# adelacvg/NS2VC

Measured on AMD Instinct MI355X. Metric: denoiser-steps/sec (10s@24kHz Vocos latent, bs32), higher is better.
Workload: dtype fp16; 1 GPU; 10 s utterance (T=938 Vocos frames), batch 32/GPU, prompt Lp=469, 20-step unipc order 2, hipGraph-captured loop, fp16 MFMA operands; timed job = set_condition + 20 steps; global_batch=32, frames=938, prompt_frames=469, solver=unipc, parallelism=dp1

## Files before the change

### include/ns2vc_hip.h

```cpp
#ifndef NS2VC_HIP_H
#define NS2VC_HIP_H

#include <stddef.h>
#include <stdint.h>

#ifdef __cplusplus
extern "C" {
#endif

#define NS2VC_ABI_VERSION 7
#define NS2VC_MAX_LEVELS 8
#define NS2VC_NCOEF 12

typedef struct ns2vc_unet ns2vc_unet;

typedef struct ns2vc_unet_cfg {
  int32_t latent_channels;
  int32_t content_channels;
  int32_t n_levels;
  int32_t block_out_channels[NS2VC_MAX_LEVELS];
  int32_t norm_num_groups;
  int32_t cross_attention_dim;
  int32_t heads;
  int32_t layers_per_block;
// ... 136 lines not shown
int ns2vc_k_xattn_pack(const void* k, int ldk, const void* v, int ldv, int B, int Lk, int hd, void* out, int precision, void* stream);

typedef struct ns2vc_geglu_args {
  const void* yn; int32_t ldy;
  const float* ln_stats; float ln_eps;
  const void* wstream; const float* consts;
  void* out_op; int32_t ldo;
  int32_t M, dim;
  unsigned* ln_health;
} ns2vc_geglu_args;
int ns2vc_pack_geglu(const float* w1_packed_host, const float* bias1_packed_host, int dim, int precision, void** out_stream_dev, float** out_consts_dev);
int ns2vc_k_geglu(const ns2vc_geglu_args* a, int precision, void* stream);
int ns2vc_pack_geglu_host(const float* w1_packed_host, const float* bias1_packed_host, int dim, int precision, uint16_t* stream_out, float* consts_out);

typedef struct ns2vc_rowchain_args {
  const void* a_op; int32_t lda;
  const void* wstream; const float* bias1; const float* consts2;
  const float* res; int32_t ldres;
  float* out1_f32; int32_t ldo1;
  void* out2_op; int32_t ldo2;
  float ln_eps; int32_t M, dim, n2;
  unsigned* ln_health;
  const float* gn_x; int32_t ldx;
  const long long* gn_stats; const float* gn_gamma; const float* gn_beta;
  float gn_eps; int32_t T, G;
  int32_t slices;
} ns2vc_rowchain_args;
int ns2vc_pack_rowchain(const float* w1_host, const float* w2_host, int dim, int n2, int precision, void** out_stream_dev);
int ns2vc_pack_rowchain_sliced(const float* w1_host, const float* w2_host, int dim, int n2, int slices, int precision, void** out_stream_dev);
int ns2vc_k_rowchain(const ns2vc_rowchain_args* a, int precision, void* stream);
int ns2vc_debug_set_geglu_min_rows(int rows);
int ns2vc_debug_set_attn_keys(int keys);
int ns2vc_debug_set_attn_optimistic(int on);
int ns2vc_debug_set_rowchain_tokens(int nt);

int ns2vc_to_operand(const float* host, size_t n, int precision, void** out_dev);
int ns2vc_from_operand(const void* dev, size_t n, int precision, float* host);
int ns2vc_round_to_operand(const float* host_in, size_t n, int precision, float* host_out);
int ns2vc_pack_weight(const float* rows_host, int N, int K, int precision, void** out_dev);
int ns2vc_k_gemm(const ns2vc_gemm_args* a, int precision, void* stream);
int ns2vc_pack_conv3_tiled(const float* rows_host, int N, int ctot, int c2, int precision, void** out_dev);
int ns2vc_weight_rowsum(const float* rows_host, int N, int K, int precision, float** out_dev);
int ns2vc_debug_set_gemm_trace(void* dev_u64_blocks_x8);
int ns2vc_debug_poison(unsigned pattern, int lds_bytes, void* stream);
int ns2vc_debug_placement(void* stream, int n_blocks, int spin, uint32_t* out_host);
int ns2vc_debug_set_gemm_tile(int bm, int bn, int stages);
int ns2vc_k_attention(const ns2vc_attn_args* a, int head_dim, int precision, void* stream);
int ns2vc_k_groupnorm(const float* a0, int lda0, int c0, const float* a1, int lda1, int c1, int B, int T, int G, float eps,
                      const float* gamma, const float* beta, const float* temb, int ldtemb, int temb_off, int silu,
                      void* out_op, void* raw_op, int precision, void* stream);
int ns2vc_k_groupnorm_stats(const float* a0, int lda0, int c0, const long long* stats0, int B, int T, int G, float eps, const float* gamma,
                            const float* beta, const float* temb, int ldtemb, int temb_off, int silu, void* out_op, int precision, void* stream);
int ns2vc_k_groupnorm_stats2(const float* a0, int lda0, int c0, const long long* stats0, const float* a1, int lda1, int c1, const long long* stats1,
                             int B, int T, int G, float eps, const float* gamma, const float* beta, const float* temb, int ldtemb, int temb_off,
                             int silu, void* out_op, void* raw_op, int precision, void* stream);
int ns2vc_k_layernorm_apply(const float* x, int ldx, int M, int C, float eps, void* out_op, int precision, void* stream);
int ns2vc_k_nct_to_btc(const float* src, int C, int T, int B, float* dst, int ldd, int cpad, void* stream);
int ns2vc_k_btc_to_nct(const float* src, int lds, int C, int T, int B, float* dst, void* stream);
int ns2vc_k_noise(const uint64_t* seeds_dev, int B, int C, int T, int ld, int step, const int32_t* lens_dev, float* out, void* stream);
int ns2vc_k_solver_update(const float* coef_dev, const int32_t* step_dev, const float* x0, float* xe, void* xe_op, int precision, float* xbar,
                          float* d1, float* mprev, float* mprev2, size_t n, int ld, void* stream);

#ifdef __cplusplus
}
#endif
#endif
// ... 1 lines not shown
```

### ns2vc_amd/_lib.py

```python
from __future__ import annotations

import ctypes as C
import os
from typing import Optional

_HERE = os.path.dirname(os.path.abspath(__file__))
LIB_PATH = os.path.join(_HERE, "lib", "libns2vc_hip.so")
NCOEF = 12
MAX_LEVELS = 8
PREC_F32, PREC_BF16, PREC_F16 = 0, 1, 2
ABI_VERSION = 7


class Ns2vcError(RuntimeError):
    pass


class UnetCfg(C.Structure):
    _fields_ = [
        ("latent_channels", C.c_int32), ("content_channels", C.c_int32), ("n_levels", C.c_int32),
        ("block_out_channels", C.c_int32 * MAX_LEVELS), ("norm_num_groups", C.c_int32),
        ("cross_attention_dim", C.c_int32), ("heads", C.c_int32), ("layers_per_block", C.c_int32),
        ("pool_heads", C.c_int32),
    ]
# ... 136 lines not shown
    "ns2vc_dev_sync": (_I, []),
    "ns2vc_stream_create": (_I, [_PP]),
    "ns2vc_stream_create_cu_mask": (_I, [_PP, C.POINTER(C.c_uint32), _I]),
    "ns2vc_stream_destroy": (_I, [_P]),
    "ns2vc_stream_sync": (_I, [_P]),
    "ns2vc_event_create": (_I, [_PP]),
    "ns2vc_event_destroy": (_I, [_P]),
    "ns2vc_event_record": (_I, [_P, _P]),
    "ns2vc_event_elapsed_ms": (_I, [_P, _P, C.POINTER(C.c_float)]),
    "ns2vc_pack_weight": (_I, [_P, _I, _I, _I, _PP]),
    "ns2vc_k_gemm": (_I, [C.POINTER(GemmArgs), _I, _P]),
    "ns2vc_pack_conv3_tiled": (_I, [_P, _I, _I, _I, _I, _PP]),
    "ns2vc_weight_rowsum": (_I, [_P, _I, _I, _I, _PP]),
    "ns2vc_debug_set_gemm_trace": (_I, [_P]),
    "ns2vc_debug_set_gemm_tile": (_I, [_I, _I, _I]),
    "ns2vc_debug_placement": (_I, [_P, _I, _I, C.POINTER(C.c_uint32)]),
    "ns2vc_debug_poison": (_I, [C.c_uint, _I, _P]),
    "ns2vc_k_attention": (_I, [C.POINTER(AttnArgs), _I, _I, _P]),
    "ns2vc_pack_ffn": (_I, [_P, _P, _I, _I, _PP]),
    "ns2vc_pack_ffn_pre": (_I, [_P, _P, _P, _I, _I, _PP]),
    "ns2vc_xattn_pack_bytes": (C.c_size_t, [_I, _I, _I]),
    "ns2vc_k_xattn_pack": (_I, [_P, _I, _P, _I, _I, _I, _I, _P, _I, _P]),
    "ns2vc_k_ffn": (_I, [C.POINTER(FfnArgs), _I, _P]),
    "ns2vc_pack_geglu": (_I, [_P, _P, _I, _I, _PP, _PP]),
    "ns2vc_k_geglu": (_I, [C.POINTER(GegluArgs), _I, _P]),
    "ns2vc_pack_geglu_host": (_I, [_P, _P, _I, _I, _P, _P]),
    "ns2vc_debug_set_geglu_min_rows": (_I, [_I]),
    "ns2vc_pack_rowchain": (_I, [_P, _P, _I, _I, _I, _PP]),
    "ns2vc_pack_rowchain_sliced": (_I, [_P, _P, _I, _I, _I, _I, _PP]),
    "ns2vc_k_rowchain": (_I, [C.POINTER(RowchainArgs), _I, _P]),
    "ns2vc_debug_set_rowchain_tokens": (_I, [_I]),
    "ns2vc_debug_set_attn_keys": (_I, [_I]),
    "ns2vc_debug_set_attn_optimistic": (_I, [_I]),
    "ns2vc_k_groupnorm_stats": (_I, [_P, _I, _I, _P, _I, _I, _I, C.c_float, _P, _P, _P, _I, _I, _I, _P, _I, _P]),
    "ns2vc_k_groupnorm_stats2": (_I, [_P, _I, _I, _P, _P, _I, _I, _P, _I, _I, _I, C.c_float, _P, _P, _P, _I, _I, _I, _P, _P, _I, _P]),
    "ns2vc_k_groupnorm": (_I, [_P, _I, _I, _P, _I, _I, _I, _I, _I, C.c_float, _P, _P, _P, _I, _I, _I, _P, _P, _I, _P]),
    "ns2vc_k_layernorm_apply": (_I, [_P, _I, _I, _I, C.c_float, _P, _I, _P]),
    "ns2vc_to_operand": (_I, [_P, C.c_size_t, _I, _PP]),
    "ns2vc_from_operand": (_I, [_P, C.c_size_t, _I, _P]),
    "ns2vc_round_to_operand": (_I, [_P, C.c_size_t, _I, _P]),
    "ns2vc_k_nct_to_btc": (_I, [_P, _I, _I, _I, _P, _I, _I, _P]),
    "ns2vc_k_btc_to_nct": (_I, [_P, _I, _I, _I, _I, _P, _P]),
    "ns2vc_k_noise": (_I, [_P, _I, _I, _I, _I, _I, _P, _P, _P]),
    "ns2vc_k_solver_update": (_I, [_P, _P, _P, _P, _P, _I, _P, _P, _P, _P, C.c_size_t, _I, _P]),
}

_lib: Optional[C.CDLL] = None


def load(path: Optional[str] = None) -> C.CDLL:
    global _lib
    if _lib is not None and path is None:
        return _lib
    p = path or os.environ.get("NS2VC_LIB") or LIB_PATH
    if not os.path.exists(p):
        raise Ns2vcError(f"{p} not found: the HIP engine is not built. Run __graft_entry__.build() "
                         f"(or `make -C ns2vc_amd/csrc`). There is no CPU fallback.")
    try:
        import torch
    except Exception:
        pass
    lib = C.CDLL(p)
    for name, (res, args) in PROTOTYPES.items():
        fn = getattr(lib, name)
        fn.restype = res
        fn.argtypes = args
# ... 12 lines not shown
```

### ns2vc_amd/csrc/attn.hip

```cpp
#include "common.h"
#include "mma.h"
#include <cstdlib>

namespace ns2vc {

template <typename T> struct AMma;
template <> struct AMma<float> {
  static constexpr int SZ = 4;
  __device__ static __forceinline__ void mma(f32x16_t& acc, const u32x4_t& a, const u32x4_t& b) {
    acc = __builtin_amdgcn_mfma_f32_32x32x2f32(__uint_as_float(a.x), __uint_as_float(b.x), acc, 0, 0, 0);
    acc = __builtin_amdgcn_mfma_f32_32x32x2f32(__uint_as_float(a.y), __uint_as_float(b.y), acc, 0, 0, 0);
    acc = __builtin_amdgcn_mfma_f32_32x32x2f32(__uint_as_float(a.z), __uint_as_float(b.z), acc, 0, 0, 0);
    acc = __builtin_amdgcn_mfma_f32_32x32x2f32(__uint_as_float(a.w), __uint_as_float(b.w), acc, 0, 0, 0);
  }
  __device__ static __forceinline__ f32x16_t mma0(const u32x4_t& a, const u32x4_t& b) {
    f32x16_t acc = __builtin_amdgcn_mfma_f32_32x32x2f32(__uint_as_float(a.x), __uint_as_float(b.x), f32x16_t{0.f, 0.f, 0.f, 0.f, 0.f, 0.f, 0.f, 0.f, 0.f, 0.f, 0.f, 0.f, 0.f, 0.f, 0.f, 0.f}, 0, 0, 0);
    acc = __builtin_amdgcn_mfma_f32_32x32x2f32(__uint_as_float(a.y), __uint_as_float(b.y), acc, 0, 0, 0);
    acc = __builtin_amdgcn_mfma_f32_32x32x2f32(__uint_as_float(a.z), __uint_as_float(b.z), acc, 0, 0, 0);
    acc = __builtin_amdgcn_mfma_f32_32x32x2f32(__uint_as_float(a.w), __uint_as_float(b.w), acc, 0, 0, 0);
    return acc;
  }
  __device__ static __forceinline__ int vpos(int key) { return key; }
};
template <typename TM> struct AMma16 {
  static constexpr int SZ = 2;
  __device__ static __forceinline__ void mma(f32x16_t& acc, const u32x4_t& a, const u32x4_t& b) { MmaT<TM>::mma(acc, a, b); }
  __device__ static __forceinline__ f32x16_t mma0(const u32x4_t& a, const u32x4_t& b) {
    f32x16_t acc = {0.f, 0.f, 0.f, 0.f, 0.f, 0.f, 0.f, 0.f, 0.f, 0.f, 0.f, 0.f, 0.f, 0.f, 0.f, 0.f};
    MmaT<TM>::mma(acc, a, b);
    return acc;
  }
  __device__ static __forceinline__ int vpos(int key) { return (key & ~12) | ((key & 4) << 1) | ((key & 8) >> 1); }
};
template <> struct AMma<bf16_t> : AMma16<bf16_t> {};
template <> struct AMma<f16_t> : AMma16<f16_t> {};

template <typename TM> __device__ __forceinline__ void vt_scatter(char* vp, int rowb, const u32x4_t& v);
template <> __device__ __forceinline__ void vt_scatter<float>(char* vp, int rowb, const u32x4_t& v) {
  *reinterpret_cast<uint32_t*>(vp) = v.x;
  *reinterpret_cast<uint32_t*>(vp + rowb) = v.y;
  *reinterpret_cast<uint32_t*>(vp + 2 * rowb) = v.z;
  *reinterpret_cast<uint32_t*>(vp + 3 * rowb) = v.w;
}
__device__ __forceinline__ void vt_scatter16(char* vp, int rowb, const u32x4_t& v) {
  *reinterpret_cast<uint16_t*>(vp) = (uint16_t)v.x;
  *reinterpret_cast<uint16_t*>(vp + rowb) = (uint16_t)(v.x >> 16);
  *reinterpret_cast<uint16_t*>(vp + 2 * rowb) = (uint16_t)v.y;
  *reinterpret_cast<uint16_t*>(vp + 3 * rowb) = (uint16_t)(v.y >> 16);
  *reinterpret_cast<uint16_t*>(vp + 4 * rowb) = (uint16_t)v.z;
  *reinterpret_cast<uint16_t*>(vp + 5 * rowb) = (uint16_t)(v.z >> 16);
  *reinterpret_cast<uint16_t*>(vp + 6 * rowb) = (uint16_t)v.w;
  *reinterpret_cast<uint16_t*>(vp + 7 * rowb) = (uint16_t)(v.w >> 16);
}
template <> __device__ __forceinline__ void vt_scatter<bf16_t>(char* vp, int rowb, const u32x4_t& v) { vt_scatter16(vp, rowb, v); }
template <> __device__ __forceinline__ void vt_scatter<f16_t>(char* vp, int rowb, const u32x4_t& v) { vt_scatter16(vp, rowb, v); }

__device__ __forceinline__ float half_max(float v) {
  const auto r = __builtin_amdgcn_permlane32_swap(__float_as_uint(v), __float_as_uint(v), false, false);
  return fmaxf(__uint_as_float(r[0]), __uint_as_float(r[1]));
}
__device__ __forceinline__ float half_sum(float v) {
  const auto r = __builtin_amdgcn_permlane32_swap(__float_as_uint(v), __float_as_uint(v), false, false);
  return __uint_as_float(r[0]) + __uint_as_float(r[1]);
}

template <typename TM> __device__ __forceinline__ float round_op(float x);
template <> __device__ __forceinline__ float round_op<float>(float x) { return x; }
template <> __device__ __forceinline__ float round_op<bf16_t>(float x) { return __uint_as_float(pack_bf16x2(0.f, x) & 0xffff0000u); }
template <> __device__ __forceinline__ float round_op<f16_t>(float x) { return f16_lo(pack_f16x2(x, 0.f)); }
template <typename TM> __device__ __forceinline__ u32x4_t aux_chunk(float e0, float e1);
template <> __device__ __forceinline__ u32x4_t aux_chunk<float>(float e0, float e1) { return u32x4_t{__float_as_uint(e0), __float_as_uint(e1), 0u, 0u}; }
template <> __device__ __forceinline__ u32x4_t aux_chunk<bf16_t>(float e0, float e1) { return u32x4_t{pack_bf16x2(e0, e1), 0u, 0u, 0u}; }
template <> __device__ __forceinline__ u32x4_t aux_chunk<f16_t>(float e0, float e1) { return u32x4_t{pack_f16x2(e0, e1), 0u, 0u, 0u}; }
template <typename TM> __device__ __forceinline__ TM op_from_float(float x);
template <> __device__ __forceinline__ float op_from_float<float>(float x) { return x; }
template <> __device__ __forceinline__ bf16_t op_from_float<bf16_t>(float x) { bf16_t r; r.v = (uint16_t)pack_bf16x2(x, 0.f); return r; }
template <> __device__ __forceinline__ f16_t op_from_float<f16_t>(float x) { f16_t r; r.v = (uint16_t)pack_f16x2(x, 0.f); return r; }

__device__ __forceinline__ uint32_t pack_fp8x4(float a, float b, float c, float d) {
  int v = __builtin_amdgcn_cvt_pk_fp8_f32(a, b, 0, false);
  v = __builtin_amdgcn_cvt_pk_fp8_f32(c, d, v, true);
  return (uint32_t)v;
}
typedef int i32x8_t __attribute__((ext_vector_type(8)));
#ifndef NS2VC_ATTN_OPT
#define NS2VC_ATTN_OPT 1
#endif
template <bool B> struct OptTag { static constexpr bool value = B; };
__device__ int g_attn_exact_only = 0;
__device__ __forceinline__ int vpos8(int key) { return ((key & 4) << 3) | ((key & 32) >> 1) | ((key & 24) >> 1) | (key & 3); }
template <typename TM, int HD, int KEYS, bool P8>
__global__ __launch_bounds__(256) void attn_kernel(const AttnArgs a) {
  op_mode_init<TM>();
  static_assert(!P8 || (sizeof(TM) == 2 && KEYS == 64), "the fp8 PV path: 16-bit operand types, one 64-key tile per f8f6f4 MFMA");
  constexpr int NSUB = KEYS / 32;
  constexpr int SZ = AMma<TM>::SZ;
  constexpr int EPC = 16 / SZ;
  constexpr int NS = HD * SZ / 32;
  constexpr int KROWB = HD * SZ + 48;
  constexpr int VSZ = P8 ? 1 : SZ;
  constexpr int VROWB = KEYS * VSZ + 16;
  constexpr int HDX = (HD + 1 + 31) / 32 * 32;
  constexpr int DT = HDX / 32;
  constexpr int NSL = SZ;
  constexpr int KBYTES = KEYS * KROWB, VBYTES = HDX * VROWB;
  constexpr int STAGE = KBYTES + VBYTES;
  constexpr int PPR = HD * SZ / 16;
  constexpr int NPIECE = KEYS * PPR;
  constexpr int UPT = (NPIECE + 255) / 256;
  constexpr float THRESH = P8 ? 8.0f : 12.0f;
  extern __shared__ __attribute__((aligned(16))) char smem[];

  const int tid = threadIdx.x, lane = tid & 63, wave = tid >> 6;
  const int l31 = lane & 31, hi = lane >> 5;
  const int nqb = (a.Lq + 127) >> 7;
  int b, h, qb;
  {
    const int nwg = gridDim.x, bid = blockIdx.x;
    const int qn = nwg >> 3, rn = nwg & 7, xcd = bid & 7, idx = bid >> 3;
    const int swz = (xcd < rn ? xcd * (qn + 1) : rn * (qn + 1) + (xcd - rn) * qn) + idx;
    b = swz / (a.H * nqb);
    const int rem = swz - b * (a.H * nqb);
    h = rem / nqb;
    qb = rem - h * nqb;
  }
  const int q = qb * 128 + wave * 32 + l31;
  const float LOG2E = 1.4426950408889634f;
  const float sc2 = a.scale * LOG2E;

  for (int i = tid * 16; i < 2 * STAGE; i += 256 * 16) *reinterpret_cast<u32x4_t*>(smem + i) = u32x4_t{0, 0, 0, 0};
  __syncthreads();
  for (int i = tid; i < 2 * KEYS; i += 256) {
    const int st = i / KEYS, key = i - st * KEYS;
    *reinterpret_cast<TM*>(smem + st * STAGE + key * KROWB + HD * SZ) = op_from_float<TM>(1.0f);
    if constexpr (P8) *reinterpret_cast<uint8_t*>(smem + st * STAGE + KBYTES + HD * VROWB + key) = (uint8_t)0x38;
    else *reinterpret_cast<TM*>(smem + st * STAGE + KBYTES + HD * VROWB + key * SZ) = op_from_float<TM>(1.0f);
  }

  u32x4_t qf[NS];
  {
    const TM* qp = reinterpret_cast<const TM*>(a.q) + ((size_t)(b * a.Lq + min(q, a.Lq - 1)) * a.ldq + h * HD);
#pragma unroll
    for (int s = 0; s < NS; ++s) {
      const u32x4_t raw = *reinterpret_cast<const u32x4_t*>(qp + s * 2 * EPC + hi * EPC);
      if constexpr (SZ == 4) {
        qf[s] = u32x4_t{__float_as_uint(__uint_as_float(raw.x) * sc2), __float_as_uint(__uint_as_float(raw.y) * sc2),
                        __float_as_uint(__uint_as_float(raw.z) * sc2), __float_as_uint(__uint_as_float(raw.w) * sc2)};
      } else {
        auto sc = [&](uint32_t w) __attribute__((always_inline)) { return Op16<TM>::pack(Op16<TM>::lo(w) * sc2, Op16<TM>::hi(w) * sc2); };
        qf[s] = u32x4_t{sc(raw.x), sc(raw.y), sc(raw.z), sc(raw.w)};
      }
      if (q >= a.Lq) qf[s] = u32x4_t{0, 0, 0, 0};
    }
  }
  float m_ref = 0.f;
  u32x4_t qaux = hi == 0 ? aux_chunk<TM>(-m_ref, 1.0f) : u32x4_t{0, 0, 0, 0};
  constexpr bool CINIT = HD == 16 && SZ == 2 && !P8;
  f32x16_t cinit;
#pragma unroll
  for (int r = 0; r < 16; ++r) cinit[r] = 0.f;

  const TM* kbase = reinterpret_cast<const TM*>(a.k) + (size_t)b * a.Lk * a.ldk + h * HD;
  const TM* vbase = reinterpret_cast<const TM*>(a.v) + (size_t)b * a.Lk * a.ldv + h * HD;
  const float* bias = a.bias ? a.bias + (size_t)b * a.Lk : nullptr;

  u32x4_t kraw[UPT], vraw[UPT];
  float braw = 0.f;
  auto load_tile = [&](int t) __attribute__((always_inline)) {
    const int key0 = t * KEYS;
#pragma unroll
    for (int i = 0; i < UPT; ++i) {
      const int u = tid + 256 * i;
      if (u < NPIECE) {
        {
          const int key = u / PPR, pc = u - key * PPR;
          const int kk = min(key0 + key, a.Lk - 1);
          kraw[i] = *reinterpret_cast<const u32x4_t*>(kbase + (size_t)kk * a.ldk + pc * EPC);
        }
        {
          const int key = u % KEYS, pc = u / KEYS;
          const int kk = min(key0 + key, a.Lk - 1);
          vraw[i] = *reinterpret_cast<const u32x4_t*>(vbase + (size_t)kk * a.ldv + pc * EPC);
        }
      }
    }
    if (tid < KEYS && bias) braw = bias[min(key0 + tid, a.Lk - 1)];
  };
  auto store_tile = [&](int stage, int key0s) __attribute__((always_inline)) {
    char* Ks = smem + stage * STAGE;
    char* Vs = Ks + KBYTES;
#pragma unroll
    for (int i = 0; i < UPT; ++i) {
      const int u = tid + 256 * i;
      if (u < NPIECE) {
        {
          const int key = u / PPR, pc = u - key * PPR;
          *reinterpret_cast<u32x4_t*>(Ks + key * KROWB + pc * 16) = kraw[i];
        }
        {
          const int key = u % KEYS, pc = u / KEYS;
          if constexpr (P8) {
            const u32x4_t w = vraw[i];
            const uint32_t b0 = pack_fp8x4(Op16<TM>::lo(w.x), Op16<TM>::hi(w.x), Op16<TM>::lo(w.y), Op16<TM>::hi(w.y));
            const uint32_t b1 = pack_fp8x4(Op16<TM>::lo(w.z), Op16<TM>::hi(w.z), Op16<TM>::lo(w.w), Op16<TM>::hi(w.w));
            uint8_t* vp = reinterpret_cast<uint8_t*>(Vs + (pc * EPC) * VROWB + vpos8(key));
#pragma unroll
            for (int j = 0; j < 4; ++j) { vp[j * VROWB] = (uint8_t)(b0 >> (8 * j)); vp[(4 + j) * VROWB] = (uint8_t)(b1 >> (8 * j)); }
          } else {
            const int pos = (key & ~31) + AMma<TM>::vpos(key & 31);
            vt_scatter<TM>(Vs + (pc * EPC) * VROWB + pos * SZ, VROWB, vraw[i]);
          }
        }
      }
    }
    if (tid < KEYS) {
      const float bl = (key0s + tid < a.Lk) ? (bias ? braw * LOG2E : 0.f) : -INFINITY;
      *reinterpret_cast<TM*>(Ks + tid * KROWB + HD * SZ + SZ) = op_from_float<TM>(bl);
    }
  };

  f32x16_t o[DT];
  const int ntile = (a.Lk + KEYS - 1) / KEYS;
  constexpr bool OPT = NS2VC_ATTN_OPT && !P8 && sizeof(TM) == 2;
  constexpr float OPT_MARGIN = 4.0f;
  auto run = [&](auto optimistic, const bool compute) __attribute__((always_inline)) {
  constexpr bool O = decltype(optimistic)::value;
  if (compute) {
#pragma unroll
    for (int d = 0; d < DT; ++d)
#pragma unroll
      for (int r = 0; r < 16; ++r) o[d][r] = 0.f;
    m_ref = 0.f;
    qaux = hi == 0 ? aux_chunk<TM>(-m_ref, 1.0f) : u32x4_t{0, 0, 0, 0};
    if constexpr (CINIT) {
#pragma unroll
      for (int r = 0; r < 16; ++r) cinit[r] = 0.f;
    }
  }
  load_tile(0);
  __syncthreads();
  store_tile(0, 0);
  __syncthreads();

  for (int t = 0; t < ntile; ++t) {
    if (t + 1 < ntile) load_tile(t + 1);
    const char* Ks = smem + (t & 1) * STAGE;
    const char* Vs = Ks + KBYTES;
    if (compute) {

    f32x16_t s[NSUB];
    if (CINIT && !bias && (t + 1 < ntile || a.Lk % KEYS == 0)) {
#pragma unroll
      for (int k2 = 0; k2 < NSUB; ++k2) {
        const char* kr = Ks + (k2 * 32 + l31) * KROWB + hi * 16;
        s[k2] = cinit;
#pragma unroll
        for (int sl = 0; sl < NS; ++sl) AMma<TM>::mma(s[k2], *reinterpret_cast<const u32x4_t*>(kr + sl * 32), qf[sl]);
      }
    } else {
#pragma unroll
    for (int k2 = 0; k2 < NSUB; ++k2) {
      const char* kr = Ks + (k2 * 32 + l31) * KROWB + hi * 16;
      s[k2] = AMma<TM>::mma0(*reinterpret_cast<const u32x4_t*>(kr + NS * 32), qaux);
#pragma unroll
      for (int sl = 0; sl < NS; ++sl) AMma<TM>::mma(s[k2], *reinterpret_cast<const u32x4_t*>(kr + sl * 32), qf[sl]);
    }
    }
    if (!O || t == 0) {
      float mx = s[0][0];
#pragma unroll
      for (int k2 = 0; k2 < NSUB; ++k2)
#pragma unroll
        for (int r = 0; r < 16; ++r) mx = fmaxf(mx, s[k2][r]);
      mx = half_max(mx);
      if (t == 0 || __any(mx > THRESH)) {
        float target = t == 0 ? mx : fmaxf(mx, 0.f);
        if (!(target > -INFINITY)) target = 0.f;
        if (O) target += OPT_MARGIN;
        const float m_new = round_op<TM>(m_ref + target);
        const float dsh = m_new - m_ref;
        if (t > 0) {
// ... 17 lines not shown
    }
#pragma unroll
    for (int k2 = 0; k2 < NSUB; ++k2)
#pragma unroll
      for (int r = 0; r < 16; ++r) s[k2][r] = __builtin_amdgcn_exp2f(s[k2][r]);

    if constexpr (P8) {
      i32x8_t pf;
#pragma unroll
      for (int v = 0; v < 8; ++v)
        pf[v] = (int)pack_fp8x4(s[v >> 2][4 * (v & 3) + 0], s[v >> 2][4 * (v & 3) + 1], s[v >> 2][4 * (v & 3) + 2], s[v >> 2][4 * (v & 3) + 3]);
#pragma unroll
      for (int d = 0; d < DT; ++d) {
        const char* vr = Vs + (d * 32 + l31) * VROWB + hi * 32;
        const u32x4_t v0 = *reinterpret_cast<const u32x4_t*>(vr), v1 = *reinterpret_cast<const u32x4_t*>(vr + 16);
        const i32x8_t vf = {(int)v0.x, (int)v0.y, (int)v0.z, (int)v0.w, (int)v1.x, (int)v1.y, (int)v1.z, (int)v1.w};
        o[d] = __builtin_amdgcn_mfma_scale_f32_32x32x64_f8f6f4(vf, pf, o[d], 0, 0, 0, 0x7f7f7f7f, 0, 0x7f7f7f7f);
      }
    } else {
#pragma unroll
    for (int k2 = 0; k2 < NSUB; ++k2) {
#pragma unroll
      for (int sl = 0; sl < NSL; ++sl) {
        u32x4_t pf;
        if constexpr (SZ == 4) {
          pf = u32x4_t{__float_as_uint(s[k2][4 * sl + 0]), __float_as_uint(s[k2][4 * sl + 1]),
                       __float_as_uint(s[k2][4 * sl + 2]), __float_as_uint(s[k2][4 * sl + 3])};
        } else {
          pf = u32x4_t{Op16<TM>::pack(s[k2][8 * sl + 0], s[k2][8 * sl + 1]), Op16<TM>::pack(s[k2][8 * sl + 2], s[k2][8 * sl + 3]),
                       Op16<TM>::pack(s[k2][8 * sl + 4], s[k2][8 * sl + 5]), Op16<TM>::pack(s[k2][8 * sl + 6], s[k2][8 * sl + 7])};
        }
#pragma unroll
        for (int d = 0; d < DT; ++d) {
          const u32x4_t vf = *reinterpret_cast<const u32x4_t*>(Vs + (d * 32 + l31) * VROWB + k2 * 32 * SZ + sl * 32 + hi * 16);
          AMma<TM>::mma(o[d], vf, pf);
        }
      }
    }
    }
    }
    if (t + 1 < ntile) store_tile((t + 1) & 1, (t + 1) * KEYS);
    __syncthreads();
  }
  };

  constexpr int LB = HD / 32, LR = ((HD % 32) / 8) * 4;
  static_assert(HD % 32 == 0 || HD % 32 == 16, "ones row must sit at row 0 or 16 of its 32-row block");
  if (OPT && !g_attn_exact_only && !a.exact_only) {
    run(OptTag<true>{}, true);
    const float lq = o[LB][LR];
    const int bad = (hi == 0 && q < a.Lq && !(lq > 0.f && lq < 16384.f)) ? 1 : 0;
    const bool wave_bad = __any(bad) != 0;
    if (__syncthreads_or(bad)) {
      if (a.fallbacks && threadIdx.x == 0) atomicAdd(a.fallbacks, 1u);
      run(OptTag<false>{}, wave_bad);
    }
  } else {
    run(OptTag<false>{}, true);
  }

  const auto lsw = __builtin_amdgcn_permlane32_swap(__float_as_uint(o[LB][LR]), __float_as_uint(o[LB][LR]), false, false);
  const float l_tot = __uint_as_float(lsw[0]);
  const float inv = 1.0f / l_tot;
  TM* op = reinterpret_cast<TM*>(a.out) + ((size_t)(b * a.Lq + min(q, a.Lq - 1)) * a.ldo + h * HD);
  if constexpr (SZ == 2) {
#pragma unroll
    for (int d = 0; d < DT; ++d)
#pragma unroll
      for (int gp = 0; gp < 2; ++gp) {
        if (d * 32 + 16 * gp < HD) {
          const uint32_t a0 = Op16<TM>::pack(o[d][8 * gp] * inv, o[d][8 * gp + 1] * inv), a1 = Op16<TM>::pack(o[d][8 * gp + 2] * inv, o[d][8 * gp + 3] * inv);
          const uint32_t b0 = Op16<TM>::pack(o[d][8 * gp + 4] * inv, o[d][8 * gp + 5] * inv), b1 = Op16<TM>::pack(o[d][8 * gp + 6] * inv, o[d][8 * gp + 7] * inv);
          const auto x0 = __builtin_amdgcn_permlane32_swap(a0, b0, false, false);
          const auto x1 = __builtin_amdgcn_permlane32_swap(a1, b1, false, false);
#if defined(NS2VC_ATTN_ABLATE_STORE)
          asm volatile("" :: "v"(x0[0]), "v"(x1[0]), "v"(x0[1]), "v"(x1[1]));
#else
          if (q < a.Lq) *reinterpret_cast<u32x4_t*>(op + d * 32 + 8 * (2 * gp + hi)) = u32x4_t{x0[0], x1[0], x0[1], x1[1]};
#endif
        }
      }
  } else if (q < a.Lq) {
#pragma unroll
    for (int d = 0; d < DT; ++d)
#pragma unroll
      for (int gq = 0; gq < 4; ++gq) {
        const int d0 = d * 32 + 8 * gq + 4 * hi;
        if (d0 < HD) store_op4<TM>(op + d0, o[d][4 * gq] * inv, o[d][4 * gq + 1] * inv, o[d][4 * gq + 2] * inv, o[d][4 * gq + 3] * inv);
      }
  }
}

template <typename TM, int HD, int KEYS> static constexpr size_t attn_lds() {
  constexpr int SZ = AMma<TM>::SZ;
  constexpr int HDX = (HD + 1 + 31) / 32 * 32;
  return 2 * (size_t)(KEYS * (HD * SZ + 48) + HDX * (KEYS * SZ + 16));
}

template <typename TM, int HD> static constexpr bool attn_has128() { return sizeof(TM) == 2 && HD <= 32; }
static int g_force_keys = 0;
void set_forced_attn_keys(int keys) { g_force_keys = keys; }
void set_attn_optimistic(int on) { const int v = on ? 0 : 1; (void)hipMemcpyToSymbol(HIP_SYMBOL(g_attn_exact_only), &v, sizeof(v)); }

template <typename TM, int HD, int KEYS> static hipError_t launch_hdk(const AttnArgs& a, hipStream_t s) {
  dim3 grid(((a.Lq + 127) / 128) * a.H * a.B);
  const size_t lds = attn_lds<TM, HD, KEYS>();
  hipLaunchKernelGGL((attn_kernel<TM, HD, KEYS, false>), grid, dim3(256), lds, s, a);
  return hipGetLastError();
}
template <typename TM, int HD> static hipError_t launch_hd(const AttnArgs& a, hipStream_t s) {
  if constexpr (sizeof(TM) == 2) {
    if (a.pv_fp8) {
      dim3 grid(((a.Lq + 127) / 128) * a.H * a.B);
      const size_t lds = attn_lds<TM, HD, 64>();
      hipLaunchKernelGGL((attn_kernel<TM, HD, 64, true>), grid, dim3(256), lds, s, a);
      return hipGetLastError();
    }
  } else if (a.pv_fp8) return hipErrorInvalidValue;
  if constexpr (attn_has128<TM, HD>()) {
    if (g_force_keys == 128) return launch_hdk<TM, HD, 128>(a, s);
  }
  return launch_hdk<TM, HD, 64>(a, s);
}

template <typename TM> static hipError_t launch_tm(const AttnArgs& a, int hd, hipStream_t s) {
  switch (hd) {
    case 16: return launch_hd<TM, 16>(a, s);
    case 32: return launch_hd<TM, 32>(a, s);
    case 48: return launch_hd<TM, 48>(a, s);
    case 64: return launch_hd<TM, 64>(a, s);
    default: return hipErrorInvalidValue;
  }
}

template <typename TM, int HD> static hipError_t set_attr() {
  hipError_t e = hipFuncSetAttribute(reinterpret_cast<const void*>(attn_kernel<TM, HD, 64, false>), hipFuncAttributeMaxDynamicSharedMemorySize,
                                     (int)attn_lds<TM, HD, 64>());
  if constexpr (attn_has128<TM, HD>()) {
    if (e == hipSuccess)
      e = hipFuncSetAttribute(reinterpret_cast<const void*>(attn_kernel<TM, HD, 128, false>), hipFuncAttributeMaxDynamicSharedMemorySize,
                              (int)attn_lds<TM, HD, 128>());
  }
  if constexpr (sizeof(TM) == 2) {
    if (e == hipSuccess)
      e = hipFuncSetAttribute(reinterpret_cast<const void*>(attn_kernel<TM, HD, 64, true>), hipFuncAttributeMaxDynamicSharedMemorySize,
                              (int)attn_lds<TM, HD, 64>());
  }
  return e;
}
template <typename TM> static hipError_t set_attr_tm() {
  hipError_t e;
  if ((e = set_attr<TM, 16>()) != hipSuccess) return e;
  if ((e = set_attr<TM, 32>()) != hipSuccess) return e;
  if ((e = set_attr<TM, 48>()) != hipSuccess) return e;
  return set_attr<TM, 64>();
}
hipError_t init_attn_attributes() {
  hipError_t e = set_attr_tm<float>();
  if (e == hipSuccess) e = set_attr_tm<bf16_t>();
  if (e == hipSuccess) e = set_attr_tm<f16_t>();
  return e;
}

hipError_t launch_attention(const AttnArgs& a, int head_dim, int prec, hipStream_t s) {
  const int al = prec == PREC_F32 ? 3 : 7;
  if (!a.q || !a.k || !a.v || !a.out) return hipErrorInvalidValue;
  if (a.Lq <= 0 || a.Lk <= 0 || (a.ldq & al) || (a.ldk & al) || (a.ldv & al) || (a.ldo & al)) return hipErrorInvalidValue;
  if (reinterpret_cast<uintptr_t>(a.out) & 15) return hipErrorInvalidValue;
  switch (prec) {
    case PREC_BF16: return launch_tm<bf16_t>(a, head_dim, s);
    case PREC_F16: return launch_tm<f16_t>(a, head_dim, s);
    case PREC_F32: return launch_tm<float>(a, head_dim, s);
    default: return hipErrorInvalidValue;
  }
}

}
```

### ns2vc_amd/csrc/common.h

```cpp
#pragma once
#include <hip/hip_runtime.h>
#include <stdint.h>
#include <stddef.h>
#include <vector>
#include "../../include/ns2vc_hip.h"

namespace ns2vc {

typedef __attribute__((ext_vector_type(8))) __bf16 bf16x8_t;
typedef __attribute__((ext_vector_type(16))) float f32x16_t;
typedef __attribute__((ext_vector_type(4))) float f32x4_t;
typedef __attribute__((ext_vector_type(4))) unsigned int u32x4_t;

struct bf16_t { uint16_t v; };
struct f16_t { uint16_t v; };

__host__ __device__ inline uint16_t f32_to_bf16_bits(float f) {
  union { float f; uint32_t u; } x;
  x.f = f;
  uint32_t u = x.u;
  if ((u & 0x7fffffffu) > 0x7f800000u) return (uint16_t)((u >> 16) | 0x40);
  u += 0x7fffu + ((u >> 16) & 1u);
  return (uint16_t)(u >> 16);
}
// ... 205 lines not shown
  sincosf(u2 * 6.2831853071795864769f, &sn, &cs);
  z0 = r * cs; z1 = r * sn;
}
__device__ __forceinline__ float4 philox_gauss4(unsigned long long seed, uint32_t t, uint32_t q, uint32_t step) {
  const uint4 x = philox4x32_10(make_uint4(t, q, step, 0u), (uint32_t)seed, (uint32_t)(seed >> 32));
  float4 z;
  box_muller(x.x, x.y, z.x, z.y);
  box_muller(x.z, x.w, z.z, z.w);
  return z;
}

constexpr double GN_SUM_SCALE = 268435456.0;
constexpr double GN_SQ_SCALE = 65536.0;

hipError_t launch_gemm(const GemmArgs& g, int prec, hipStream_t s);
size_t xattn_pack_bytes(int B, int Lk, int hd);
hipError_t launch_xattn_pack(const void* k, int ldk, const void* v, int ldv, int B, int Lk, int hd, void* out, int prec, hipStream_t s);
bool gemm_uses_convts(const GemmArgs& g, int prec);
int last_gemm_refusal_line();
hipError_t launch_attention(const AttnArgs& a, int head_dim, int prec, hipStream_t s);
hipError_t init_gemm_attributes();
bool convts_eligible(const GemmArgs& g, int prec);
int convts_default_bn(const GemmArgs& g);
int convts_bn_for(const GemmArgs& g, int bn128_min);
void set_convts_bn128_min(int wgs);
int convts_row_blocks(const GemmArgs& g);
hipError_t launch_convts(const GemmArgs& g, int prec, int bn, int nl, int ks, hipStream_t s);
hipError_t init_convts_attributes();
hipError_t pack_conv3_tiled(const float* rows, int N, int ctot, int c2, int prec, std::vector<unsigned char>& out);
void set_forced_gemm_tile(int bm, int bn, int stages);
void set_gemm_trace(unsigned long long* p);
hipError_t init_attn_attributes();
void set_forced_attn_keys(int keys);
hipError_t launch_ffn(const ::ns2vc_ffn_args& a, int prec, hipStream_t s);
bool ffn_eligible(int dim, int T, int prec);
hipError_t init_ffn_attributes();

hipError_t launch_gn_partial(const float* a0, int lda0, int c0, const float* a1, int lda1, int c1,
                             int B, int T, int G, double* partial, int nchunk, int rows_per_chunk, hipStream_t s);
hipError_t launch_gn_apply(const float* a0, int lda0, int c0, const float* a1, int lda1, int c1, int B, int T, int G, float eps,
                           const double* partial, int nchunk, const long long* st0, const long long* st1, const float* gamma,
                           const float* beta, const float* temb, int ldtemb, int temb_off, int silu, void* out_op, void* raw_op,
                           int prec, hipStream_t s, int pair = 0,
                           const int* lens = nullptr);
hipError_t launch_mask_rows(void* dst, size_t ldd_bytes, size_t row_bytes, int B, int T, const int* lens, hipStream_t s, const void* src = nullptr,
                            size_t lds_bytes = 0, int Tsrc = 0, int up = 0);
hipError_t launch_ln_apply_op(const float* x, int ldx, int M, int C, float eps, void* out_op, int prec, hipStream_t s);
hipError_t launch_cast_op(const float* x, size_t n, void* out_op, int prec, hipStream_t s, int split = 0);
hipError_t launch_time_embed(const float* t_ptr, int t_stride, const int* step_ptr, int coef_stride,
                             const float* w1t, const float* b1, const float* w2t, const float* b2,
                             const float* aug, float* emb, void* emb_act_op, int prec, int B, int tdim, int edim, hipStream_t s);
hipError_t launch_rowchain(const ::ns2vc_rowchain_args& a, int prec, hipStream_t s);
bool rowchain_eligible(int dim, int n2, int T, int prec);
hipError_t init_rowchain_attributes();
void set_forced_rowchain_tokens(int nt);
hipError_t launch_emb_from_table(const float* table, const int* step_ptr, const float* aug, float* emb, void* emb_act_op, int prec, int B,
                                 int edim, hipStream_t s);
int probe_xcd_round_robin(unsigned* map8 = nullptr);
hipError_t launch_zero(void* p, size_t bytes, hipStream_t s, int* counter = nullptr);
hipError_t launch_copy16(const void* src, void* dst, size_t bytes, hipStream_t s);
hipError_t launch_poison(unsigned pattern, int lds_bytes, unsigned* sink, hipStream_t s);
hipError_t launch_nct_to_btc(const float* src, int C, int T, int B, float* dst_f32, void* dst_op, int prec, int ldd, int cpad, hipStream_t s,
                             int ldd_op = 0, int split = 0);
hipError_t launch_btc_to_nct(const float* src, int lds, int C, int T, int B, float* dst, hipStream_t s);
hipError_t launch_mask_bias(const uint8_t* mask, int n, float* bias, hipStream_t s);
hipError_t launch_ln_apply(const float* x, int M, int C, float eps, const float* gamma, const float* beta,
// ... 18 lines not shown
```

### ns2vc_amd/csrc/engine.cpp

```cpp
#include "common.h"

#include <algorithm>
#include <cmath>
#include <cstdarg>
#include <cstdio>
#include <cstring>
#include <cstdlib>
#include <functional>
#include <map>
#include <memory>
#include <string>
#include <vector>
#include <mutex>

using namespace ns2vc;

namespace ns2vc {
hipError_t pack_ffn_stream(const float* w1p, const float* w2f, const float* w0, int dim, int prec, std::vector<unsigned short>& out);
hipError_t pack_rowchain_stream(const float* w1, const float* w2, int dim, int n2, int prec, std::vector<unsigned short>& out, int slices = 1);
int rowchain_slice_blocks(int n2, int slices);
void set_ffn_trace(unsigned long long* p);
typedef ::ns2vc_geglu_args GegluArgs;
bool geglu_eligible(int dim, int T, int prec);
hipError_t pack_geglu_stream(const float* w1p, const float* bias1p, int dim, int prec, std::vector<unsigned short>& stream, std::vector<float>& consts);
// ... 2274 lines not shown
    inited = true;
  }
  std::vector<unsigned short> st;
  if (pack_rowchain_stream(w1_host, w2_host, dim, n2, precision, st) != hipSuccess)
    return fail("rowchain: dim must be 128, 256 or 384, n2 = dim or 3 dim, and the precision 16-bit");
  void* d = nullptr;
  HIPCHK(hipMalloc(&d, st.size() * 2));
  HIPCHK(hipMemcpy(d, st.data(), st.size() * 2, hipMemcpyHostToDevice));
  *out_stream_dev = d;
  return 0;
}
int ns2vc_pack_rowchain_sliced(const float* w1_host, const float* w2_host, int dim, int n2, int slices, int precision, void** out_stream_dev) {
  if (!w1_host || !w2_host || !out_stream_dev) return fail("null argument");
  static bool inited = false;
  if (!inited) {
    hipError_t e = init_rowchain_attributes();
    if (e != hipSuccess) return fail("kernel attribute setup failed: %s", hipGetErrorString(e));
    inited = true;
  }
  std::vector<unsigned short> st;
  if (pack_rowchain_stream(w1_host, w2_host, dim, n2, precision, st, slices) != hipSuccess)
    return fail("rowchain (sliced): dim 384, n2 = dim or 3 dim, 2 slices, 16-bit precision");
  void* d = nullptr;
  HIPCHK(hipMalloc(&d, st.size() * 2));
  HIPCHK(hipMemcpy(d, st.data(), st.size() * 2, hipMemcpyHostToDevice));
  *out_stream_dev = d;
  return 0;
}
int ns2vc_debug_set_attn_keys(int keys) {
  if (keys != 0 && keys != 64 && keys != 128) return fail("attention K/V tile: 0 (heuristic), 64 or 128 keys");
  set_forced_attn_keys(keys);
  return 0;
}
int ns2vc_debug_set_rowchain_tokens(int nt) {
  if (nt < 0 || nt > 2) return fail("rowchain tokens: 0 (heuristic), 1 (64-token blocks) or 2 (128-token blocks)");
  set_forced_rowchain_tokens(nt);
  return 0;
}
int ns2vc_k_rowchain(const ns2vc_rowchain_args* a, int precision, void* stream) {
  if (!a) return fail("null args");
  hipError_t e = launch_rowchain(*a, precision, (hipStream_t)stream);
  if (e != hipSuccess) return fail("launch_rowchain: %s", hipGetErrorString(e));
  return 0;
}
size_t ns2vc_xattn_pack_bytes(int B, int Lk, int hd) { return xattn_pack_bytes(B, Lk, hd); }
int ns2vc_k_xattn_pack(const void* k, int ldk, const void* v, int ldv, int B, int Lk, int hd, void* out, int precision, void* stream) {
  hipError_t e = launch_xattn_pack(k, ldk, v, ldv, B, Lk, hd, out, precision, (hipStream_t)stream);
  if (e != hipSuccess) return fail("xattn_pack: %s (16-bit precisions, head dim 16 | 32, 8 heads, 16-byte aligned k rows)", hipGetErrorString(e));
  return 0;
}
int ns2vc_k_ffn(const ns2vc_ffn_args* a, int precision, void* stream) {
  if (!a) return fail("null args");
  hipError_t e = launch_ffn(*a, precision, (hipStream_t)stream);
  if (e != hipSuccess) return fail("launch_ffn: %s", hipGetErrorString(e));
  return 0;
}
int ns2vc_pack_geglu(const float* w1_packed_host, const float* bias1_packed_host, int dim, int precision, void** out_stream_dev, float** out_consts_dev) {
  if (!w1_packed_host || !out_stream_dev || !out_consts_dev) return fail("null argument");
  hipError_t e = init_geglu_attributes();
  if (e != hipSuccess) return fail("kernel attribute setup failed: %s", hipGetErrorString(e));
  std::vector<unsigned short> st;
  std::vector<float> cs;
  if (pack_geglu_stream(w1_packed_host, bias1_packed_host, dim, precision, st, cs) != hipSuccess) return fail("geglu: dim must be 384 and the precision 16-bit");
  void* d = nullptr;
  float* c = nullptr;
  HIPCHK(hipMalloc(&d, st.size() * 2));
// ... 129 lines not shown
```

Measured before the change: 294.9 denoiser-steps/s (batch 32 per GPU, whole job).

## Store V row-major in LDS and read transposed via ds_read_tr16

Adds a row-major, XOR-swizzled V image in shared memory for 16-bit attention, read with the transposing LDS load (ds_read_tr16_b64) to build MFMA B operands. This replaces the transposing scatter into a column-major V tile during staging, aiming to cut store-side bank conflicts and scatter instructions. For head dim 16 with 64-key tiles it also stages 128 keys per pipeline step, halving barrier and load-store rounds at the cost of more LDS per block. It is on by default, with a debug toggle to fall back.

```diff
diff --git a/include/ns2vc_hip.h b/include/ns2vc_hip.h
--- a/include/ns2vc_hip.h
+++ b/include/ns2vc_hip.h
@@ -192,6 +192,7 @@
 int ns2vc_debug_set_geglu_min_rows(int rows);
 int ns2vc_debug_set_attn_keys(int keys);
 int ns2vc_debug_set_attn_optimistic(int on);
+int ns2vc_debug_set_attn_vimage(int on);
 int ns2vc_debug_set_rowchain_tokens(int nt);
 
 int ns2vc_to_operand(const float* host, size_t n, int precision, void** out_dev);
diff --git a/ns2vc_amd/_lib.py b/ns2vc_amd/_lib.py
--- a/ns2vc_amd/_lib.py
+++ b/ns2vc_amd/_lib.py
@@ -192,6 +192,7 @@
     "ns2vc_debug_set_rowchain_tokens": (_I, [_I]),
     "ns2vc_debug_set_attn_keys": (_I, [_I]),
     "ns2vc_debug_set_attn_optimistic": (_I, [_I]),
+    "ns2vc_debug_set_attn_vimage": (_I, [_I]),
     "ns2vc_k_groupnorm_stats": (_I, [_P, _I, _I, _P, _I, _I, _I, C.c_float, _P, _P, _P, _I, _I, _I, _P, _I, _P]),
     "ns2vc_k_groupnorm_stats2": (_I, [_P, _I, _I, _P, _P, _I, _I, _P, _I, _I, _I, C.c_float, _P, _P, _P, _I, _I, _I, _P, _P, _I, _P]),
     "ns2vc_k_groupnorm": (_I, [_P, _I, _I, _P, _I, _I, _I, _I, _I, C.c_float, _P, _P, _P, _I, _I, _I, _P, _P, _I, _P]),
diff --git a/ns2vc_amd/csrc/attn.hip b/ns2vc_amd/csrc/attn.hip
--- a/ns2vc_amd/csrc/attn.hip
+++ b/ns2vc_amd/csrc/attn.hip
@@ -54,6 +54,21 @@
 }
 template <> __device__ __forceinline__ void vt_scatter<bf16_t>(char* vp, int rowb, const u32x4_t& v) { vt_scatter16(vp, rowb, v); }
 template <> __device__ __forceinline__ void vt_scatter<f16_t>(char* vp, int rowb, const u32x4_t& v) { vt_scatter16(vp, rowb, v); }
+
+template <int ROWB> __device__ __forceinline__ int vimg_chunk(int key, int c) {
+  if constexpr (ROWB == 64) return c ^ (key & 2);
+  else if constexpr (ROWB == 128) return c ^ (((key ^ (key >> 1)) & 1) << 2) ^ (key & 2);
+  else return c;
+}
+typedef short i16x4_t __attribute__((ext_vector_type(4)));
+typedef uint32_t u32x2_t __attribute__((ext_vector_type(2)));
+__device__ __forceinline__ u32x2_t lds_read_tr16(const char* p) {
+  return __builtin_bit_cast(u32x2_t, __builtin_amdgcn_ds_read_tr16_b64_v4i16((__attribute__((address_space(3))) i16x4_t*)(p)));
+}
+#ifndef NS2VC_ATTN_STAGE128
+#define NS2VC_ATTN_STAGE128 1
+#endif
+template <int HD, int KEYS, bool VI> constexpr int attn_stage_keys() { return NS2VC_ATTN_STAGE128 && VI && HD == 16 && KEYS == 64 ? 128 : KEYS; }
 
 __device__ __forceinline__ float half_max(float v) {
   const auto r = __builtin_amdgcn_permlane32_swap(__float_as_uint(v), __float_as_uint(v), false, false);
@@ -89,10 +104,11 @@
 template <bool B> struct OptTag { static constexpr bool value = B; };
 __device__ int g_attn_exact_only = 0;
 __device__ __forceinline__ int vpos8(int key) { return ((key & 4) << 3) | ((key & 32) >> 1) | ((key & 24) >> 1) | (key & 3); }
-template <typename TM, int HD, int KEYS, bool P8>
+template <typename TM, int HD, int KEYS, bool P8, bool VI>
 __global__ __launch_bounds__(256) void attn_kernel(const AttnArgs a) {
   op_mode_init<TM>();
   static_assert(!P8 || (sizeof(TM) == 2 && KEYS == 64), "the fp8 PV path: 16-bit operand types, one 64-key tile per f8f6f4 MFMA");
+  static_assert(!VI || (sizeof(TM) == 2 && !P8), "the row-major V image: 16-bit operand types, not the fp8 PV path");
   constexpr int NSUB = KEYS / 32;
   constexpr int SZ = AMma<TM>::SZ;
   constexpr int EPC = 16 / SZ;
@@ -103,10 +119,12 @@
   constexpr int HDX = (HD + 1 + 31) / 32 * 32;
   constexpr int DT = HDX / 32;
   constexpr int NSL = SZ;
-  constexpr int KBYTES = KEYS * KROWB, VBYTES = HDX * VROWB;
+  constexpr int STG = attn_stage_keys<HD, KEYS, VI>();
+  constexpr int VIROWB = HDX * SZ;
+  constexpr int KBYTES = STG * KROWB, VBYTES = VI ? STG * VIROWB : HDX * VROWB;
   constexpr int STAGE = KBYTES + VBYTES;
   constexpr int PPR = HD * SZ / 16;
-  constexpr int NPIECE = KEYS * PPR;
+  constexpr int NPIECE = STG * PPR;
   constexpr int UPT = (NPIECE + 255) / 256;
   constexpr float THRESH = P8 ? 8.0f : 12.0f;
   extern __shared__ __attribute__((aligned(16))) char smem[];
@@ -130,10 +148,11 @@
 
   for (int i = tid * 16; i < 2 * STAGE; i += 256 * 16) *reinterpret_cast<u32x4_t*>(smem + i) = u32x4_t{0, 0, 0, 0};
   __syncthreads();
-  for (int i = tid; i < 2 * KEYS; i += 256) {
-    const int st = i / KEYS, key = i - st * KEYS;
+  for (int i = tid; i < 2 * STG; i += 256) {
+    const int st = i / STG, key = i - st * STG;
     *reinterpret_cast<TM*>(smem + st * STAGE + key * KROWB + HD * SZ) = op_from_float<TM>(1.0f);
-    if constexpr (P8) *reinterpret_cast<uint8_t*>(smem + st * STAGE + KBYTES + HD * VROWB + key) = (uint8_t)0x38;
+    if constexpr (VI) *reinterpret_cast<TM*>(smem + st * STAGE + KBYTES + key * VIROWB + vimg_chunk<VIROWB>(key, PPR) * 16) = op_from_float<TM>(1.0f);
+    else if constexpr (P8) *reinterpret_cast<uint8_t*>(smem + st * STAGE + KBYTES + HD * VROWB + key) = (uint8_t)0x38;
     else *reinterpret_cast<TM*>(smem + st * STAGE + KBYTES + HD * VROWB + key * SZ) = op_from_float<TM>(1.0f);
   }
 
@@ -166,8 +185,16 @@
 
   u32x4_t kraw[UPT], vraw[UPT];
   float braw = 0.f;
+  auto vi_piece = [&](int u, int& key, int& pc) __attribute__((always_inline)) {
+    if constexpr (PPR == 6) {
+      if (u < 4 * STG) { key = u >> 2; pc = u & 3; }
+      else { key = (u - 4 * STG) >> 1; pc = 4 + (u & 1); }
+    } else {
+      key = u / PPR; pc = u - key * PPR;
+    }
+  };
   auto load_tile = [&](int t) __attribute__((always_inline)) {
-    const int key0 = t * KEYS;
+    const int key0 = t * STG;
 #pragma unroll
     for (int i = 0; i < UPT; ++i) {
       const int u = tid + 256 * i;
@@ -178,13 +205,15 @@
           kraw[i] = *reinterpret_cast<const u32x4_t*>(kbase + (size_t)kk * a.ldk + pc * EPC);
         }
         {
-          const int key = u % KEYS, pc = u / KEYS;
+          int key, pc;
+          if constexpr (VI) vi_piece(u, key, pc);
+          else { key = u % KEYS; pc = u / KEYS; }
           const int kk = min(key0 + key, a.Lk - 1);
           vraw[i] = *reinterpret_cast<const u32x4_t*>(vbase + (size_t)kk * a.ldv + pc * EPC);
         }
       }
     }
-    if (tid < KEYS && bias) braw = bias[min(key0 + tid, a.Lk - 1)];
+    if (tid < STG && bias) braw = bias[min(key0 + tid, a.Lk - 1)];
   };
   auto store_tile = [&](int stage, int key0s) __attribute__((always_inline)) {
     char* Ks = smem + stage * STAGE;
@@ -197,7 +226,11 @@
           const int key = u / PPR, pc = u - key * PPR;
           *reinterpret_cast<u32x4_t*>(Ks + key * KROWB + pc * 16) = kraw[i];
         }
-        {
+        if constexpr (VI) {
+          int key, pc;
+          vi_piece(u, key, pc);
+          *reinterpret_cast<u32x4_t*>(Vs + key * VIROWB + vimg_chunk<VIROWB>(key, pc) * 16) = vraw[i];
+        } else {
           const int key = u % KEYS, pc = u / KEYS;
           if constexpr (P8) {
             const u32x4_t w = vraw[i];
@@ -213,7 +246,7 @@
         }
       }
     }
-    if (tid < KEYS) {
+    if (tid < STG) {
       const float bl = (key0s + tid < a.Lk) ? (bias ? braw * LOG2E : 0.f) : -INFINITY;
       *reinterpret_cast<TM*>(Ks + tid * KROWB + HD * SZ + SZ) = op_from_float<TM>(bl);
     }
@@ -221,6 +254,14 @@
 
   f32x16_t o[DT];
   const int ntile = (a.Lk + KEYS - 1) / KEYS;
+  const int nstg = (a.Lk + STG - 1) / STG;
+  int voff[DT];
+  if constexpr (VI) {
+    const int qr = (lane & 15) >> 2, pp = lane & 3;
+#pragma unroll
+    for (int d = 0; d < DT; ++d)
+      voff[d] = (4 * hi + qr) * VIROWB + vimg_chunk<VIROWB>(qr, d * 4 + 2 * ((lane >> 4) & 1) + (pp >> 1)) * 16 + 8 * (pp & 1);
+  }
   constexpr bool OPT = NS2VC_ATTN_OPT && !P8 && sizeof(TM) == 2;
   constexpr float OPT_MARGIN = 4.0f;
   auto run = [&](auto optimistic, const bool compute) __attribute__((always_inline)) {
@@ -242,11 +283,14 @@
   store_tile(0, 0);
   __syncthreads();
 
-  for (int t = 0; t < ntile; ++t) {
-    if (t + 1 < ntile) load_tile(t + 1);
-    const char* Ks = smem + (t & 1) * STAGE;
-    const char* Vs = Ks + KBYTES;
-    if (compute) {
+  for (int sg = 0; sg < nstg; ++sg) {
+    if (sg + 1 < nstg) load_tile(sg + 1);
+#pragma unroll 1
+  for (int j = 0; j < STG / KEYS; ++j) {
+    const int t = sg * (STG / KEYS) + j;
+    const char* Ks = smem + (sg & 1) * STAGE + j * KEYS * KROWB;
+    const char* Vs = smem + (sg & 1) * STAGE + KBYTES + j * KEYS * VIROWB;
+    if (compute && (STG == KEYS || t < ntile)) {
 
     f32x16_t s[NSUB];
     if (CINIT && !bias && (t + 1 < ntile || a.Lk % KEYS == 0)) {
@@ -330,14 +374,21 @@
         }
 #pragma unroll
         for (int d = 0; d < DT; ++d) {
-          const u32x4_t vf = *reinterpret_cast<const u32x4_t*>(Vs + (d * 32 + l31) * VROWB + k2 * 32 * SZ + sl * 32 + hi * 16);
-          AMma<TM>::mma(o[d], vf, pf);
-        }
-      }
-    }
-    }
-    }
-    if (t + 1 < ntile) store_tile((t + 1) & 1, (t + 1) * KEYS);
+          if constexpr (VI) {
+            const char* vr = Vs + voff[d] + (k2 * 32 + 16 * sl) * VIROWB;
+            const u32x2_t v0 = lds_read_tr16(vr), v1 = lds_read_tr16(vr + 8 * VIROWB);
+            AMma<TM>::mma(o[d], u32x4_t{v0.x, v0.y, v1.x, v1.y}, pf);
+          } else {
+            const u32x4_t vf = *reinterpret_cast<const u32x4_t*>(Vs + (d * 32 + l31) * VROWB + k2 * 32 * SZ + sl * 32 + hi * 16);
+            AMma<TM>::mma(o[d], vf, pf);
+          }
+        }
+      }
+    }
+    }
+    }
+  }
+    if (sg + 1 < nstg) store_tile((sg + 1) & 1, (sg + 1) * STG);
     __syncthreads();
   }
   };
@@ -389,29 +440,42 @@
   }
 }
 
-template <typename TM, int HD, int KEYS> static constexpr size_t attn_lds() {
+template <typename TM, int HD, int KEYS, bool VI> static constexpr size_t attn_lds() {
   constexpr int SZ = AMma<TM>::SZ;
   constexpr int HDX = (HD + 1 + 31) / 32 * 32;
-  return 2 * (size_t)(KEYS * (HD * SZ + 48) + HDX * (KEYS * SZ + 16));
+  constexpr int STG = attn_stage_keys<HD, KEYS, VI>();
+  return 2 * (size_t)(STG * (HD * SZ + 48) + (VI ? STG * HDX * SZ : HDX * (KEYS * SZ + 16)));
 }
 
 template <typename TM, int HD> static constexpr bool attn_has128() { return sizeof(TM) == 2 && HD <= 32; }
 static int g_force_keys = 0;
 void set_forced_attn_keys(int keys) { g_force_keys = keys; }
 void set_attn_optimistic(int on) { const int v = on ? 0 : 1; (void)hipMemcpyToSymbol(HIP_SYMBOL(g_attn_exact_only), &v, sizeof(v)); }
+#ifndef NS2VC_ATTN_VIMAGE
+#define NS2VC_ATTN_VIMAGE 1
+#endif
+static int g_attn_vimage = NS2VC_ATTN_VIMAGE;
+void set_attn_vimage(int on) { g_attn_vimage = on ? 1 : 0; }
 
 template <typename TM, int HD, int KEYS> static hipError_t launch_hdk(const AttnArgs& a, hipStream_t s) {
   dim3 grid(((a.Lq + 127) / 128) * a.H * a.B);
-  const size_t lds = attn_lds<TM, HD, KEYS>();
-  hipLaunchKernelGGL((attn_kernel<TM, HD, KEYS, false>), grid, dim3(256), lds, s, a);
+  if constexpr (sizeof(TM) == 2) {
+    if (g_attn_vimage) {
+      const size_t lds = attn_lds<TM, HD, KEYS, true>();
+      hipLaunchKernelGGL((attn_kernel<TM, HD, KEYS, false, true>), grid, dim3(256), lds, s, a);
+      return hipGetLastError();
+    }
+  }
+  const size_t lds = attn_lds<TM, HD, KEYS, false>();
+  hipLaunchKernelGGL((attn_kernel<TM, HD, KEYS, false, false>), grid, dim3(256), lds, s, a);
   return hipGetLastError();
 }
 template <typename TM, int HD> static hipError_t launch_hd(const AttnArgs& a, hipStream_t s) {
   if constexpr (sizeof(TM) == 2) {
     if (a.pv_fp8) {
       dim3 grid(((a.Lq + 127) / 128) * a.H * a.B);
-      const size_t lds = attn_lds<TM, HD, 64>();
-      hipLaunchKernelGGL((attn_kernel<TM, HD, 64, true>), grid, dim3(256), lds, s, a);
+      const size_t lds = attn_lds<TM, HD, 64, false>();
+      hipLaunchKernelGGL((attn_kernel<TM, HD, 64, true, false>), grid, dim3(256), lds, s, a);
       return hipGetLastError();
     }
   } else if (a.pv_fp8) return hipErrorInvalidValue;
@@ -431,18 +495,19 @@
   }
 }
 
+template <typename TM, int HD, int KEYS, bool P8, bool VI> static hipError_t set_attr1() {
+  return hipFuncSetAttribute(reinterpret_cast<const void*>(attn_kernel<TM, HD, KEYS, P8, VI>), hipFuncAttributeMaxDynamicSharedMemorySize,
+                             (int)attn_lds<TM, HD, KEYS, VI>());
+}
 template <typename TM, int HD> static hipError_t set_attr() {
-  hipError_t e = hipFuncSetAttribute(reinterpret_cast<const void*>(attn_kernel<TM, HD, 64, false>), hipFuncAttributeMaxDynamicSharedMemorySize,
-                                     (int)attn_lds<TM, HD, 64>());
+  hipError_t e = set_attr1<TM, HD, 64, false, false>();
   if constexpr (attn_has128<TM, HD>()) {
-    if (e == hipSuccess)
-      e = hipFuncSetAttribute(reinterpret_cast<const void*>(attn_kernel<TM, HD, 128, false>), hipFuncAttributeMaxDynamicSharedMemorySize,
-                              (int)attn_lds<TM, HD, 128>());
+    if (e == hipSuccess) e = set_attr1<TM, HD, 128, false, false>();
+    if (e == hipSuccess) e = set_attr1<TM, HD, 128, false, true>();
   }
   if constexpr (sizeof(TM) == 2) {
-    if (e == hipSuccess)
-      e = hipFuncSetAttribute(reinterpret_cast<const void*>(attn_kernel<TM, HD, 64, true>), hipFuncAttributeMaxDynamicSharedMemorySize,
-                              (int)attn_lds<TM, HD, 64>());
+    if (e == hipSuccess) e = set_attr1<TM, HD, 64, false, true>();
+    if (e == hipSuccess) e = set_attr1<TM, HD, 64, true, false>();
   }
   return e;
 }
diff --git a/ns2vc_amd/csrc/common.h b/ns2vc_amd/csrc/common.h
--- a/ns2vc_amd/csrc/common.h
+++ b/ns2vc_amd/csrc/common.h
@@ -261,6 +261,7 @@
 void set_gemm_trace(unsigned long long* p);
 hipError_t init_attn_attributes();
 void set_forced_attn_keys(int keys);
+void set_attn_vimage(int on);
 hipError_t launch_ffn(const ::ns2vc_ffn_args& a, int prec, hipStream_t s);
 bool ffn_eligible(int dim, int T, int prec);
 hipError_t init_ffn_attributes();
diff --git a/ns2vc_amd/csrc/engine.cpp b/ns2vc_amd/csrc/engine.cpp
--- a/ns2vc_amd/csrc/engine.cpp
+++ b/ns2vc_amd/csrc/engine.cpp
@@ -2330,6 +2330,10 @@
   set_forced_attn_keys(keys);
   return 0;
 }
+int ns2vc_debug_set_attn_vimage(int on) {
+  set_attn_vimage(on);
+  return 0;
+}
 int ns2vc_debug_set_rowchain_tokens(int nt) {
   if (nt < 0 || nt > 2) return fail("rowchain tokens: 0 (heuristic), 1 (64-token blocks) or 2 (128-token blocks)");
   set_forced_rowchain_tokens(nt);
```

Result: no change. 297.3 denoiser-steps/s (batch 32 per GPU, whole job) (median of 6 runs) (+0.8%).
